# honglianghe/CDNet

Measured on AMD Instinct MI355X. Metric: tiles/sec (train fwd+bwd+Adam), 256x256, higher is better.
Workload: dtype fp32

## Files before the change

cdnet_amd/csrc/conv32.hip:

```cpp
#include <type_traits>
#include "common.h"
#include "conv_args.h"
#include "launch.h"
#include <stdlib.h>

using namespace cdnet;

typedef __attribute__((ext_vector_type(8))) __bf16 bf16x8;
typedef __attribute__((ext_vector_type(2))) __bf16 bf16x2;
typedef __attribute__((ext_vector_type(16))) float f32x16;
typedef __attribute__((ext_vector_type(2))) float f32x2;
typedef unsigned u32x4 __attribute__((ext_vector_type(4)));
typedef float f32x4 __attribute__((ext_vector_type(4)));

namespace {

__device__ __forceinline__ void split8(const float *v, u32x4 &hi, u32x4 &lo) {
#pragma unroll
    for (int k = 0; k < 4; ++k) {
        const f32x2 x = {v[2 * k], v[2 * k + 1]};
        const bf16x2 h = __builtin_convertvector(x, bf16x2);
        const unsigned hb = __builtin_bit_cast(unsigned, h);
        const f32x2 hf = {__builtin_bit_cast(float, hb << 16), __builtin_bit_cast(float, hb & 0xffff0000u)};
        const bf16x2 l = __builtin_convertvector(x - hf, bf16x2);
// ... 328 lines not shown
                        const float v = acc[mi][ni][r];
                        ssum[ni] += v;
                        ssq[ni] = fmaf(v, v, ssq[ni]);
                    }
            } else {
#pragma unroll
            for (int mi = 0; mi < MPW; ++mi)
#pragma unroll
                for (int r = 0; r < 16; ++r) {
                    const int m = (wm * MPW + mi) * 32 + (r & 3) + 8 * (r >> 2) + 4 * half;
                    const float v = ((y0 + m / TW) < A.H && (x0 + m % TW) < A.W) ? acc[mi][ni][r] : 0.f;
                    ssum[ni] += v;
                    ssq[ni] = fmaf(v, v, ssq[ni]);
                }
            }
            ssum[ni] += __shfl_xor(ssum[ni], 32);
            ssq[ni] += __shfl_xor(ssq[ni], 32);
            if (half == 0) {
                s_stats[wave][0][(wn * NPW + ni) * 32 + l31] = ssum[ni];
                s_stats[wave][1][(wn * NPW + ni) * 32 + l31] = ssq[ni];
            }
        }
        __syncthreads();
        if (tid < 2 * BN) {
            const int which = tid / BN, col = tid % BN;
            const int wn_of = col / (NPW * 32);
            float v = 0.f;
#pragma unroll
            for (int k = 0; k < WM; ++k) v += s_stats[k * WN + wn_of][which][col];
            const int co = cout0 + col;
            if (co < A.Cout) A.stats[((size_t)tile * 2 + which) * A.Cout + co] = v;
        }
    }
    store_tile_f32<MPW, NPW, TW>(A, acc, n, y0, x0, wm * MPW, wn * NPW, half, l31, cout0, par >> 1, par & 1);
}

template <int TH, int TW, int BN, int WM, int WN, int TAPS>
int launch_conv32(const ConvArgs &A, hipStream_t st) {
    using L = Lds32<TH, TW, BN, TAPS>;
    int ctot = 0;
    for (int i = 0; i < A.nsrc; ++i) ctot += A.src[i].C;
    const int smem = L::bytes(ctot);
    dim3 grid(cdiv(A.W, TW) * cdiv(A.H, TH) * A.N * A.npar, cdiv(A.Cout, BN), 1);
    return launch_lds<conv_f32_kernel<TH, TW, BN, WM, WN, TAPS>>(grid, 256, L::bytes(XF_MAX), smem, st, "hipFuncSetAttribute(conv32)", "conv_f32_kernel", A);
}

template <int TAPS>
int dispatch_conv32(const ConvArgs &A, hipStream_t st) {
    if (A.tile == 16 && A.BN == 64) return launch_conv32<16, 16, 64, 4, 1, TAPS>(A, st);
    if (A.tile == 16 && A.BN == 32) return launch_conv32<16, 16, 32, 4, 1, TAPS>(A, st);
    if (A.tile == 8 && A.BN == 64) return launch_conv32<8, 8, 64, 2, 2, TAPS>(A, st);
    set_error("cdnet_conv_forward(f32): unsupported configuration tile=%d CK=%d BN=%d", A.tile, A.CK, A.BN);
    return CDNET_E_ARG;
}

template <int BN, int NCH, bool XF, bool ERES>
__global__ __launch_bounds__(256, 4) void conv1x1_f32_stream_kernel(ConvArgs A) {
    constexpr int NPW = BN / 32;
    constexpr int B_PLANE = CK * BN * 2;
    constexpr int CIN = NCH * CK;
    __shared__ __attribute__((aligned(16))) unsigned char smem[NCH * 2 * B_PLANE + 2 * CIN * 4];
    unsigned char *lds_b = smem;
    float *s_xf = reinterpret_cast<float *>(smem + NCH * 2 * B_PLANE);

    const int tid = threadIdx.x, lane = tid & 63, wave = __builtin_amdgcn_readfirstlane(tid >> 6);
    const int half = lane >> 5, l31 = lane & 31;
    const int cout_tile = blockIdx.y, cout0 = cout_tile * BN;
    const ConvSrc &S = A.src[0];
    {
        const u32x4 *wsrc = reinterpret_cast<const u32x4 *>(A.w + (size_t)cout_tile * NCH * B_PLANE);
        u32x4 *bdst = reinterpret_cast<u32x4 *>(lds_b);
        for (int v = tid; v < NCH * 2 * B_PLANE / 16; v += 256) bdst[v] = wsrc[v];
        for (int c = tid; c < CIN; c += 256) {
            s_xf[c] = S.scale ? S.scale[c] : 1.f;
            s_xf[CIN + c] = S.shift ? S.shift[c] : 0.f;
        }
    }
    __syncthreads();

    const size_t P = (size_t)A.N * A.H * A.W;
    const int nblk = (int)((P + 31) / 32), bstride = (int)gridDim.x * 4;
    int blk = (int)blockIdx.x * 4 + wave;
    if (blk >= nblk) return;
    const bool relu = S.relu != 0, orelu = A.orelu != 0, eres_relu = A.eres_relu != 0;
    const int cout = A.Cout;
    const int bbase = half * BN * 16 + l31 * 16;

    float osc[NPW], osh[NPW], esc[NPW], esh[NPW];
#pragma unroll
    for (int ni = 0; ni < NPW; ++ni) {
        const int co = cout0 + ni * 32 + l31, c = co < A.Cout ? co : 0;
        osc[ni] = A.oscale ? A.oscale[c] : 1.f;
        osh[ni] = fmaf(A.bias ? A.bias[c] : 0.f, osc[ni], A.oshift ? A.oshift[c] : 0.f);
        esc[ni] = (ERES && A.eres_scale) ? A.eres_scale[c] : 1.f;
        esh[ni] = (ERES && A.eres_shift) ? A.eres_shift[c] : 0.f;
    }

    const char *xbase = reinterpret_cast<const char *>(S.x);
    char *obase = reinterpret_cast<char *>(A.out) + (size_t)A.out_coff * 4;
    const char *ebase = ERES ? reinterpret_cast<const char *>(A.eres) : xbase;
    const unsigned cs4 = (unsigned)A.out_cstride * 4, ce4 = (unsigned)cout * 4;
    const unsigned vo_in = l31 * (CIN * 4) + half * 32;
    unsigned vo_out[NPW], vo_eres[NPW];
#pragma unroll
    for (int ni = 0; ni < NPW; ++ni) {
        const unsigned co = cout0 + ni * 32 + l31;
// ... 154 lines not shown
        auto xf = [&](float4 v, const float4 *r) {
            v.x = fmaf(v.x, sc.x, sh.x); v.y = fmaf(v.y, sc.y, sh.y); v.z = fmaf(v.z, sc.z, sh.z); v.w = fmaf(v.w, sc.w, sh.w);
            if (r) { v.x += r->x; v.y += r->y; v.z += r->z; v.w += r->w; }
            if (relu) { v.x = fmaxf(v.x, 0.f); v.y = fmaxf(v.y, 0.f); v.z = fmaxf(v.z, 0.f); v.w = fmaxf(v.w, 0.f); }
            return v;
        };
        if (ys >= 0 && ys < Hl && xs >= 0 && xs < Wl) {
            if (!s.pool) {
                const size_t e = img + (size_t)ys * rs + (size_t)xs * s.C + c;
                const float4 raw = *reinterpret_cast<const float4 *>(sx + e);
                if (sr) { const float4 r = *reinterpret_cast<const float4 *>(sr + e); val = xf(raw, &r); }
                else val = xf(raw, nullptr);
            } else {
                float4 raw[4];
                bool ok[4];
#pragma unroll
                for (int q = 0; q < 4; ++q) {
                    int yy = 2 * ys + (q >> 1), xx = 2 * xs + (q & 1);
                    ok[q] = q == 0 || (yy < s.Hs && xx < s.Ws);
                    yy = yy < s.Hs ? yy : s.Hs - 1;
                    xx = xx < s.Ws ? xx : s.Ws - 1;
                    raw[q] = *reinterpret_cast<const float4 *>(sx + img + (size_t)yy * rs + (size_t)xx * s.C + c);
                }
#pragma unroll
                for (int q = 0; q < 4; ++q) {
                    const float4 t = xf(raw[q], nullptr);
                    if (q == 0) val = t;
                    else if (ok[q]) { val.x = fmaxf(val.x, t.x); val.y = fmaxf(val.y, t.y); val.z = fmaxf(val.z, t.z); val.w = fmaxf(val.w, t.w); }
                }
            }
        }
        *reinterpret_cast<float4 *>(out + pix * s.C + c) = val;
    }
}

}

namespace cdnet {

int conv_forward_f32(const ConvArgs &A, hipStream_t st) {
    CDNET_REQUIRE(A.CK == 16, "cdnet_conv_forward(f32): CK must be 16 (got %d)", A.CK);
    for (int i = 0; i < A.nsrc; ++i)
        CDNET_REQUIRE(!A.src[i].pool, "cdnet_conv_forward(f32): pooled sources must be materialised (cdnet_src_materialize)");
    CDNET_REQUIRE(!A.out_f16, "cdnet_conv_forward(f32): out_f16 must be 0");
    {
        const int rc = conv_forward_f32_ws(A, st);
        if (rc >= 0) return rc;
    }
    CDNET_REQUIRE(A.ws != 2, "cdnet_conv_forward(f32): the BatchNorm-backward statistics epilogue (ws = 2) needs the producer / consumer kernel "
                             "(ask cdnet_conv_ws_eligible first)");
    CDNET_REQUIRE(A.taps1 == 0 || A.taps1 == A.taps, "cdnet_conv_forward(f32): a one-tap second source runs on conv_ws32_kernel only (ask cdnet_conv_ws_eligible)");
    CDNET_REQUIRE(!A.pool_out, "cdnet_conv_forward(f32): the fused max-pool output rides in conv_ws32_kernel's epilogue only (ask cdnet_conv_ws_eligible)");
    if (A.taps == 9) return dispatch_conv32<9>(A, st);
    if (A.taps == 4) return dispatch_conv32<4>(A, st);
    {
        const int rc = try_conv1x1_stream(A, st);
        if (rc >= 0) return rc;
    }
    return dispatch_conv32<1>(A, st);
}

int materialize_f32(const ConvSrc &s, int N, int H, int W, void *out, hipStream_t st) {
    const size_t total = (size_t)N * H * W * (s.C / 4);
    size_t g = (total + 255) / 256;
    g = g > 8192 ? 8192 : g;
    materialize_f32_kernel<<<(int)g, 256, 0, st>>>(s, N, H, W, reinterpret_cast<float *>(out));
    return check_launch("cdnet_src_materialize(f32)");
}

}
```

cdnet_amd/csrc/conv_args.h:

```cpp
#pragma once
#include "../../include/cdnet_hip.h"

struct ConvSrc {
    const unsigned short *x;
    const unsigned short *res;
    const float *scale;
    const float *shift;
    int C, Hs, Ws, pool, relu, off_y, off_x;
    int f16, row_stride;
};

struct ConvArgs {
    ConvSrc src[2];
    int nsrc;
    const unsigned short *w;
    const float *bias;
    const float *oscale;
    const float *oshift;
    int orelu;
    unsigned short *out;
    int Cout, out_cstride, out_coff;
    float *stats;
    int N, H, W;
    int taps, npar, ostride, nchunk;
    int tile, CK, BN;
    int out_f16;
    int debug;
    int ws;
    int f32;
    const unsigned short *eres;
    const float *eres_scale, *eres_shift;
    int eres_f16, eres_relu;
    int taps1, pad_;
    unsigned short *pool_out;
    const float *dot_w, *dot_b;
    float *dot_out;
};

enum : int {
    CONV_DBG_WS16_QUAD = 16,
    CONV_DBG_ONE_TILE = 32,
    CONV_DBG_PERSIST_SMALL = 64,
    CONV_DBG_OLD_WS16 = 128,
    CONV_DBG_NO_STREAM_1X1 = 256,
    CONV_DBG_GRID_SHIFT = 8,
};
enum : int {
    WGRAD_DBG_NO_WS = 8,
    WGRAD_DBG_ALL_QUADS = 16,
};

static_assert(sizeof(ConvSrc) == sizeof(cdnet_conv_src), "ConvSrc layout");
static_assert(sizeof(ConvArgs) == sizeof(cdnet_conv_args), "ConvArgs layout");

namespace cdnet {
int conv_forward_f32(const ConvArgs &A, hipStream_t st);
int conv_forward_f32_ws(const ConvArgs &A, hipStream_t st, bool dry_run = false);
int conv_forward_ws16(const ConvArgs &A, hipStream_t st, bool dry_run = false);
int materialize_f32(const ConvSrc &s, int N, int H, int W, void *out, hipStream_t st);
}
```

cdnet_amd/csrc/conv.hip:

```cpp
#include <type_traits>
#include <vector>
#include "common.h"
#include "conv_args.h"
#include "launch.h"
#include "xform.h"
#include "stage16.h"
#include <stdlib.h>

using namespace cdnet;

typedef __attribute__((ext_vector_type(16))) float f32x16;
typedef __attribute__((ext_vector_type(4))) float f32x4;

namespace {

__device__ int g_dbg_dummy;

struct PackDesc {
    const float *w;
    unsigned short *out;
    int Cout, Cin, KH, KW, CK, BN, nchunk, ntile, TAPS, mode, parity;
    unsigned block0, nblocks;
    int split;
    const float *scale;
};

__device__ __forceinline__ void pack_range(const PackDesc &d, size_t first, size_t stride) {
    const float *__restrict__ w = d.w;
    unsigned short *__restrict__ out = d.out;
    const int Cout = d.Cout, Cin = d.Cin, KH = d.KH, KW = d.KW, CK = d.CK, BN = d.BN, nchunk = d.nchunk, TAPS = d.TAPS, mode = d.mode,
              parity = d.parity;
    const size_t total = (size_t)d.ntile * nchunk * TAPS * (CK / 16) * 2 * BN * (d.split ? 2 : 1);
    for (size_t i = first; i < total; i += stride) {
        size_t r = i;
        int tap = r % TAPS; r /= TAPS;
        int col = r % BN; r /= BN;
        int half = r % 2; r /= 2;
        int kc = r % (CK / 16); r /= (CK / 16);
        int hl = 0;
        if (d.split) { hl = r % 2; r /= 2; }
        int chunk = r % nchunk; r /= nchunk;
        int tile = (int)r;
        int co = tile * BN + col;
        const size_t ovec = ((((((size_t)tile * nchunk + chunk) * (d.split ? 2 : 1) + hl) * TAPS + tap) * (CK / 16) + kc) * 2 + half) * BN + col;
        unsigned short o8[8];
#pragma unroll
        for (int j = 0; j < 8; ++j) {
        int ci = chunk * CK + kc * 16 + half * 8 + j;
        float v = 0.f;
        if (co < Cout && ci < Cin) {
            if (mode == 0) {
                v = w[(((size_t)co * Cin + ci) * KH + tap / KW) * KW + tap % KW];
            } else if (mode == 1) {
                int kh = KH - 1 - tap / KW, kw = KW - 1 - tap % KW;
                v = w[(((size_t)ci * Cout + co) * KH + kh) * KW + kw];
            } else if (mode == 2) {
                int a = parity >> 1, b = parity & 1, ty = tap >> 1, tx = tap & 1;
                int kh = a == 0 ? (ty == 0 ? 1 : 3) : (ty == 0 ? 0 : 2);
                int kw = b == 0 ? (tx == 0 ? 1 : 3) : (tx == 0 ? 0 : 2);
                v = w[(((size_t)ci * Cout + co) * 4 + kh) * 4 + kw];
            } else if (mode == 3) {
                int a = parity >> 1, b = parity & 1;
                v = w[(((size_t)ci * Cout + co) * 2 + a) * 2 + b];
            } else if (mode == 7) {
                const int Ct = Cout / 4;
                const int a = co / (2 * Ct), b = (co / Ct) & 1, c = co % Ct;
                const int tf = 8 - tap;
                const int kh = 2 * (tf / 3 - 1) + a + 1, kw = 2 * (tf % 3 - 1) + b + 1;
                if (kh >= 0 && kh < 3 && kw >= 0 && kw < 3) v = w[(((size_t)ci * Ct + c) * 3 + kh) * 3 + kw];
            } else {
                const int Ct = Cin / 4;
                const int a = ci / (2 * Ct), b = (ci / Ct) & 1, c = ci % Ct;
                if (mode == 4) {
                    const int kh = 2 * (tap / 3) + a - 1, kw = 2 * (tap % 3) + b - 1;
                    if (kh >= 0 && kh < 4 && kw >= 0 && kw < 4) v = w[(((size_t)co * Ct + c) * 4 + kh) * 4 + kw];
                } else if (mode == 5) {
                    v = w[(((size_t)co * Ct + c) * 2 + a) * 2 + b];
                } else {
                    const int kh = 2 * (tap / 3 - 1) + a + 1, kw = 2 * (tap % 3 - 1) + b + 1;
                    if (kh >= 0 && kh < 3 && kw >= 0 && kw < 3) v = w[(((size_t)co * Ct + c) * 3 + kh) * 3 + kw];
                }
            }
        }
        if (d.scale && co < Cout) v *= d.scale[co];
        const unsigned short hi = f2bf(v);
        o8[j] = hl ? f2bf(v - bf2f(hi)) : hi;
        }
        uint4 ov;
        ov.x = o8[0] | ((unsigned)o8[1] << 16); ov.y = o8[2] | ((unsigned)o8[3] << 16);
        ov.z = o8[4] | ((unsigned)o8[5] << 16); ov.w = o8[6] | ((unsigned)o8[7] << 16);
        reinterpret_cast<uint4 *>(out)[ovec] = ov;
    }
}

__global__ void pack_weights_kernel(PackDesc d) {
    pack_range(d, (size_t)blockIdx.x * blockDim.x + threadIdx.x, (size_t)gridDim.x * blockDim.x);
}

__global__ void pack_weights_batch_kernel(const PackDesc *__restrict__ table, int n) {
    int lo = 0, hi = n - 1;
    while (lo < hi) {
        const int mid = (lo + hi + 1) >> 1;
        if (table[mid].block0 <= blockIdx.x) lo = mid; else hi = mid - 1;
    }
    const PackDesc d = table[lo];
    pack_range(d, (size_t)(blockIdx.x - d.block0) * blockDim.x + threadIdx.x, (size_t)d.nblocks * blockDim.x);
}

__device__ __forceinline__ V16 max8(V16 a, V16 b, bool nonneg) {
    V16 o;
    if (nonneg) {
        o.u = __builtin_bit_cast(uint4, xf_max_nonneg_bf8(__builtin_bit_cast(xf_u32x4, a.u), __builtin_bit_cast(xf_u32x4, b.u)));
        return o;
    }
#pragma unroll
    for (int j = 0; j < 8; ++j) o.h[j] = bf2f(a.h[j]) >= bf2f(b.h[j]) ? a.h[j] : b.h[j];
    return o;
}

constexpr int XF_MAX = 2048;

__device__ __forceinline__ void load_chan_xf(ChanXf &t, const ConvSrc &s, const float *xf, int xfs, int c) {
    t.on = s.scale != nullptr;
    if (!t.on) return;
    const float4 *ps = reinterpret_cast<const float4 *>(xf ? xf + c : s.scale + c);
    const float4 *ph = reinterpret_cast<const float4 *>(xf ? xf + xfs + c : s.shift + c);
    float4 a = ps[0], b = ps[1], cc = ph[0], d = ph[1];
    t.sc[0] = a.x; t.sc[1] = a.y; t.sc[2] = a.z; t.sc[3] = a.w; t.sc[4] = b.x; t.sc[5] = b.y; t.sc[6] = b.z; t.sc[7] = b.w;
    t.sh[0] = cc.x; t.sh[1] = cc.y; t.sh[2] = cc.z; t.sh[3] = cc.w; t.sh[4] = d.x; t.sh[5] = d.y; t.sh[6] = d.z; t.sh[7] = d.w;
}

template <int TH, int CK>
struct HaloImg {
    static constexpr bool SWZ = (TH == 16 && CK == 16);
    static constexpr int PSTR = SWZ ? CK * 2 : CK * 2 + 16;
    __device__ __forceinline__ static int off(int pix, int hy, int slot) { return pix * PSTR + (SWZ ? ((slot ^ (hy & 1)) * 16) : slot * 16); }
};

template <int TH, int TW, int CK>
__device__ __forceinline__ void stage_input(const ConvSrc &s, int cc0, int n, int y0, int x0, int H, int W,
                                            unsigned char *lds_a, int tid, const float *xf = nullptr, int xfs = 0) {
    constexpr int VPP = CK / 8;
    constexpr int HW_ = TW + 2, NPIX = (TH + 2) * (TW + 2);
    const int slot = tid % VPP;
    ChanXf t;
    load_chan_xf(t, s, xf, xfs, cc0 + slot * 8);
    const bool relu = s.relu != 0;
    const bool f16 = s.f16 != 0;
    const bool plain = !t.on && !relu && s.res == nullptr && !f16;
    const int Hl = s.pool ? (s.Hs + (s.pool == 2)) / 2 : s.Hs, Wl = s.pool ? (s.Ws + (s.pool == 2)) / 2 : s.Ws;
    const size_t rs = s.row_stride ? (size_t)s.row_stride : (size_t)s.Ws * s.C;
    const size_t img = (size_t)n * s.Hs * rs;
    for (int v = tid; v < NPIX * VPP; v += 256) {
        const int pix = v / VPP;
        const int hy = pix / HW_, hx = pix - hy * HW_;
        const int y = y0 - 1 + hy, x = x0 - 1 + hx;
        V16 val;
        val.u = make_uint4(0, 0, 0, 0);
        const int ys = y - s.off_y, xs = x - s.off_x;
// ... 1056 lines not shown
__global__ __launch_bounds__(256) void materialize_kernel(const ConvSrc s, int N, int H, int W, unsigned short *__restrict__ out) {
    const int VPP = s.C / 8;
    const size_t total = (size_t)N * H * W * VPP;
    const bool relu = s.relu != 0, f16 = s.f16 != 0;
    const int Hl = s.pool ? (s.Hs + (s.pool == 2)) / 2 : s.Hs, Wl = s.pool ? (s.Ws + (s.pool == 2)) / 2 : s.Ws;
    const size_t rs = s.row_stride ? (size_t)s.row_stride : (size_t)s.Ws * s.C;
    for (size_t i = (size_t)blockIdx.x * 256 + threadIdx.x; i < total; i += (size_t)gridDim.x * 256) {
        const int slot = (int)(i % VPP);
        const size_t pix = i / VPP;
        const int x = (int)(pix % W), y = (int)((pix / W) % H), n = (int)(pix / ((size_t)W * H));
        ChanXf t;
        load_chan_xf(t, s, nullptr, 0, slot * 8);
        const bool plain = !t.on && !relu && s.res == nullptr && !f16;
        const size_t img = (size_t)n * s.Hs * rs;
        V16 val;
        val.u = make_uint4(0, 0, 0, 0);
        const int ys = y - s.off_y, xs = x - s.off_x;
        if (ys >= 0 && ys < Hl && xs >= 0 && xs < Wl) {
            if (!s.pool) {
                const size_t e = img + (size_t)ys * rs + (size_t)xs * s.C + slot * 8;
                V16 raw;
                raw.u = *reinterpret_cast<const uint4 *>(s.x + e);
                if (plain) val = raw;
                else if (s.res) { V16 r; r.u = *reinterpret_cast<const uint4 *>(s.res + e); val = xform8(raw, &r, t, relu, f16); }
                else val = xform8(raw, nullptr, t, relu, f16);
            } else {
                V16 raw[4];
                bool ok[4];
#pragma unroll
                for (int q = 0; q < 4; ++q) {
                    int yy = 2 * ys + (q >> 1), xx = 2 * xs + (q & 1);
                    ok[q] = q == 0 || (yy < s.Hs && xx < s.Ws);
                    yy = yy < s.Hs ? yy : s.Hs - 1;
                    xx = xx < s.Ws ? xx : s.Ws - 1;
                    raw[q].u = *reinterpret_cast<const uint4 *>(s.x + img + (size_t)yy * rs + (size_t)xx * s.C + slot * 8);
                }
#pragma unroll
                for (int q = 0; q < 4; ++q) {
                    const V16 tv = plain ? raw[q] : xform8(raw[q], nullptr, t, relu, f16);
                    val = q == 0 ? tv : (ok[q] ? max8(val, tv, relu) : val);
                }
            }
        }
        *reinterpret_cast<uint4 *>(out + pix * s.C + slot * 8) = val.u;
    }
}

}

extern "C" size_t cdnet_conv_packed_weight_elems(int Cout, int Cin_padded_chunks, int taps, int CK, int BN, int npar) {
    return (size_t)npar * cdiv(Cout, BN) * Cin_padded_chunks * taps * CK * BN;
}

static int fill_pack_desc(PackDesc &d, const float *w, void *packed, int Cout, int Cin, int KH, int KW, int CK, int BN, int mode, int p,
                          const char *who) {
    const int split = (mode & 16) ? 1 : 0;
    mode &= 15;
    CDNET_REQUIRE(w && packed, "%s: null pointer", who);
    CDNET_REQUIRE(CK % 16 == 0 && BN % 32 == 0 && Cin % CK == 0 && mode >= 0 && mode <= 7, "%s: Cin=%d CK=%d BN=%d mode=%d", who, Cin, CK, BN, mode);
    const int taps = mode == 2 ? 4 : (mode == 3 ? 1 : ((mode == 4 || mode == 6 || mode == 7) ? 9 : (mode == 5 ? 1 : KH * KW)));
    const int nchunk = Cin / CK, ntile = cdiv(Cout, BN);
    const size_t per = (size_t)ntile * nchunk * taps * CK * BN * (split ? 2 : 1);
    d.split = split;
    d.scale = nullptr;
    d.w = w; d.out = (unsigned short *)packed + (size_t)p * per;
    d.Cout = Cout; d.Cin = Cin; d.KH = KH; d.KW = KW; d.CK = CK; d.BN = BN; d.nchunk = nchunk; d.ntile = ntile; d.TAPS = taps; d.mode = mode;
    d.parity = p;
    d.block0 = 0;
    d.nblocks = (unsigned)((per + 2047) / 2048);
    if (d.nblocks > 4096) d.nblocks = 4096;
    return CDNET_OK;
}

extern "C" int cdnet_pack_conv_weights(const float *w, void *packed, int Cout, int Cin, int KH, int KW, int CK, int BN,
                                       int mode, void *stream) {
    const int npar = ((mode & 15) == 2 || (mode & 15) == 3) ? 4 : 1;
    for (int p = 0; p < npar; ++p) {
        PackDesc d;
        int rc = fill_pack_desc(d, w, packed, Cout, Cin, KH, KW, CK, BN, mode, p, "cdnet_pack_conv_weights");
        if (rc) return rc;
        pack_weights_kernel<<<d.nblocks, 256, 0, (hipStream_t)stream>>>(d);
    }
    return check_launch("cdnet_pack_conv_weights");
}

extern "C" int cdnet_pack_conv_weights_scaled(const float *w, const float *cout_scale, void *packed, int Cout, int Cin, int KH, int KW, int CK,
                                              int BN, int mode, void *stream) {
    CDNET_REQUIRE(cout_scale && (mode & 15) == 0, "cdnet_pack_conv_weights_scaled: forward Conv2d packs (mode 0) with a scale vector");
    PackDesc d;
    int rc = fill_pack_desc(d, w, packed, Cout, Cin, KH, KW, CK, BN, mode, 0, "cdnet_pack_conv_weights_scaled");
    if (rc) return rc;
    d.scale = cout_scale;
    pack_weights_kernel<<<d.nblocks, 256, 0, (hipStream_t)stream>>>(d);
    return check_launch("cdnet_pack_conv_weights_scaled");
}

extern "C" size_t cdnet_pack_batch_table_bytes(int n_jobs) { return (size_t)n_jobs * 4 * sizeof(PackDesc); }

extern "C" int cdnet_pack_conv_weights_batch(const cdnet_pack_job *jobs, int n_jobs, void *table, size_t table_bytes, int upload,
                                             void *stream) {
    CDNET_REQUIRE(jobs && n_jobs > 0 && table, "cdnet_pack_conv_weights_batch: null pointer / no jobs");
    CDNET_REQUIRE(table_bytes >= cdnet_pack_batch_table_bytes(n_jobs), "cdnet_pack_conv_weights_batch: table too small");
    static thread_local std::vector<PackDesc> host;
    host.clear();
    unsigned blocks = 0;
    for (int j = 0; j < n_jobs; ++j) {
        const cdnet_pack_job &J = jobs[j];
        const int npar = ((J.mode & 15) == 2 || (J.mode & 15) == 3) ? 4 : 1;
        for (int p = 0; p < npar; ++p) {
            PackDesc d;
            int rc = fill_pack_desc(d, J.w, J.packed, J.Cout, J.Cin, J.KH, J.KW, J.CK, J.BN, J.mode, p, "cdnet_pack_conv_weights_batch");
            if (rc) return rc;
            d.block0 = blocks;
            blocks += d.nblocks;
            host.push_back(d);
        }
    }
    hipStream_t st = (hipStream_t)stream;
    if (upload) {
        if (hipMemcpyAsync(table, host.data(), host.size() * sizeof(PackDesc), hipMemcpyHostToDevice, st) != hipSuccess ||
            hipStreamSynchronize(st) != hipSuccess)
            return check_launch("cdnet_pack_conv_weights_batch(upload)");
    }
    pack_weights_batch_kernel<<<blocks, 256, 0, st>>>((const PackDesc *)table, (int)host.size());
    return check_launch("cdnet_pack_conv_weights_batch");
}

extern "C" int cdnet_conv_forward(const cdnet_conv_args *args, void *stream) {
    CDNET_REQUIRE(args, "cdnet_conv_forward: null args");
    const ConvArgs &A = *reinterpret_cast<const ConvArgs *>(args);
    CDNET_REQUIRE(A.nsrc >= 1 && A.nsrc <= 2 && A.w && (A.out || A.dot_out), "cdnet_conv_forward: bad pointers / nsrc=%d", A.nsrc);
    CDNET_REQUIRE(!A.dot_out || (A.dot_w && !A.f32 && !A.pool_out), "cdnet_conv_forward: dot_out needs dot_w, the 16-bit path and no pool_out");
    CDNET_REQUIRE(A.N > 0 && A.H > 0 && A.W > 0 && A.Cout > 0 && A.Cout % 8 == 0, "cdnet_conv_forward: bad size (Cout must be a multiple of 8)");
    {
        int ctot_xf = 0;
        for (int i = 0; i < A.nsrc; ++i) ctot_xf += A.src[i].C;
        CDNET_REQUIRE(ctot_xf <= XF_MAX, "cdnet_conv_forward: %d source channels exceed the %d-entry scale/shift table", ctot_xf, XF_MAX);
    }
    CDNET_REQUIRE(A.ws == 0 || A.ws == 2, "cdnet_conv_forward: ws must be 0 or 2 (BatchNorm-backward statistics epilogue)");
    if (A.f32) {
        CDNET_REQUIRE(A.f32 == 1, "cdnet_conv_forward: f32 must be 0 or 1");
        for (int i = 0; i < A.nsrc; ++i)
            CDNET_REQUIRE(A.src[i].f16 == 2, "cdnet_conv_forward(f32): every source must be fp32 (f16 = 2)");
    } else {
        for (int i = 0; i < A.nsrc; ++i)
            CDNET_REQUIRE(A.src[i].f16 == 0 || A.src[i].f16 == 1, "cdnet_conv_forward: fp32 sources need args.f32 = 1");
    }
    if (A.eres && A.ws != 2) {
        CDNET_REQUIRE(A.ostride == 1 && A.npar == 1 && A.out_coff == 0 && A.out_cstride == A.Cout && !A.stats && !A.orelu &&
                      !A.out_f16 && ((A.eres_scale == nullptr) == (A.eres_shift == nullptr)),
                      "cdnet_conv_forward: fused residual epilogue needs a dense bf16 output, no statistics and no ReLU before the add");
    }
    int nchunk = 0;
    for (int i = 0; i < A.nsrc; ++i) {
        CDNET_REQUIRE(A.src[i].x && A.src[i].C % A.CK == 0, "cdnet_conv_forward: source %d channels %d not a multiple of CK=%d",
                      i, A.src[i].C, A.CK);
        CDNET_REQUIRE(!(A.src[i].pool && A.src[i].res), "cdnet_conv_forward: pool+residual source unsupported");
        nchunk += A.src[i].C / A.CK;
    }
    const bool padded = A.nchunk == nchunk + 1 && A.taps == 9 && A.nsrc == 2 && !A.f32;
    CDNET_REQUIRE(nchunk == A.nchunk || padded, "cdnet_conv_forward: nchunk %d != %d", A.nchunk, nchunk);
    CDNET_REQUIRE((A.taps == 9 && A.npar == 1 && A.ostride == 1) || (A.taps == 1 && A.npar == 1 && A.ostride == 1) ||
                  (A.taps == 4 && A.npar == 4 && A.ostride == 2) || (A.taps == 1 && A.npar == 4 && A.ostride == 2),
                  "cdnet_conv_forward: taps=%d npar=%d ostride=%d", A.taps, A.npar, A.ostride);
// ... 54 lines not shown
```

include/cdnet_hip.h:

```cpp
#ifndef CDNET_HIP_H
#define CDNET_HIP_H

#include <stddef.h>
#include <stdint.h>

#ifdef __cplusplus
extern "C" {
#endif

#define CDNET_OK            0
#define CDNET_E_ARG         1
#define CDNET_E_WORKSPACE   2
#define CDNET_E_LAUNCH      3

#define CDNET_ABI_VERSION   5

int         cdnet_abi_version(void);
size_t      cdnet_abi_sizeof(const char *struct_name);
const char *cdnet_last_error(void);
const char *cdnet_build_info(void);
int         cdnet_spin(int microseconds, void *stream);
int         cdnet_box_copy(const void *src, void *dst, size_t bytes, void *stream);
int         cdnet_box_mfma(const uint32_t *seed, float *sink, unsigned long long *stamps, int workgroups, int waves_per_wg, int iters, void *stream);

// ... 35 lines not shown
                             float *prob, uint8_t *pred, uint8_t *fill, uint8_t *small, int32_t *label, int32_t *final_, int32_t *counts,
                             void *stream);
int cdnet_dilate_labels(const int32_t *label, int N, int H, int W, int radius, int32_t *out, void *stream);


typedef struct cdnet_conv_src {
    const uint16_t *x;
    const uint16_t *res;
    const float *scale;
    const float *shift;
    int C;
    int Hs, Ws;
    int pool;
    int relu;
    int off_y, off_x;
    int f16;
    int row_stride;
} cdnet_conv_src;

typedef struct cdnet_conv_args {
    cdnet_conv_src src[2];
    int nsrc;
    const uint16_t *w;
    const float *bias;
    const float *oscale;
    const float *oshift;
    int orelu;
    uint16_t *out;
    int Cout, out_cstride, out_coff;
    float *stats;
    int N, H, W;
    int taps;
    int npar;
    int ostride;
    int nchunk;
    int tile, CK, BN;
    int out_f16;
    int debug;
    int ws;
    int f32;
    const uint16_t *eres;
    const float *eres_scale, *eres_shift;
    int eres_f16, eres_relu;
    int taps1;
    int pad_;
    uint16_t *pool_out;
    const float *dot_w;
    const float *dot_b;
    float *dot_out;
} cdnet_conv_args;

size_t cdnet_conv_packed_weight_elems(int Cout, int nchunk, int taps, int CK, int BN, int npar);
#define CDNET_PACK_SPLIT 16
int cdnet_pack_conv_weights(const float *w, void *packed, int Cout, int Cin, int KH, int KW, int CK, int BN, int mode,
                            void *stream);
int cdnet_pack_conv_weights_scaled(const float *w, const float *cout_scale, void *packed, int Cout, int Cin, int KH, int KW, int CK,
                                   int BN, int mode, void *stream);
typedef struct cdnet_pack_job {
    const float *w;
    void *packed;
    int Cout, Cin, KH, KW, CK, BN, mode, pad_;
} cdnet_pack_job;
size_t cdnet_pack_batch_table_bytes(int n_jobs);
int cdnet_pack_conv_weights_batch(const cdnet_pack_job *jobs, int n_jobs, void *table, size_t table_bytes, int upload,
                                  void *stream);
int cdnet_conv_forward(const cdnet_conv_args *args, void *stream);

int cdnet_input_pack(const float *x, int N, int C, int H, int W, void *out_bf16_nhwc16, void *stream);
int cdnet_input_pack_f32(const float *x, int N, int C, int H, int W, float *out_f32_nhwc16, void *stream);
int cdnet_bn_fold_eval(const float *gamma, const float *beta, const float *running_mean, const float *running_var,
                       const float *conv_bias, float eps, int C, float *scale, float *shift, void *stream);
int cdnet_bn_finalize_train(const float *stats, int T, int C, float count, const float *gamma, const float *beta,
                            const float *conv_bias, float eps, float momentum, float *running_mean,
                            float *running_var, float *scale, float *shift, float *save_mean, float *save_invstd,
                            void *stream);

typedef struct cdnet_head_feat {
    const uint16_t *raw;
    const uint16_t *res;
    const float *scale;
    const float *shift;
    int relu;
    int f16;
} cdnet_head_feat;

#define CDNET_HEAD_WEIGHT_FLOATS 855
int cdnet_dam_head_forward(const cdnet_head_feat *f1, const cdnet_head_feat *f2, const cdnet_head_feat *f3,
                           const float *head_weights, int N, int H, int W, float *mask, float *point,
                           float *direction, void *stream);
int cdnet_final_conv1x1(const cdnet_head_feat *f, const float *w, const float *b, int K, int N, int H, int W,
                        float *out, void *stream);
size_t cdnet_bias_grad_workspace_floats(int C);
int cdnet_bias_grad(const uint16_t *grad_out, size_t npix, int C, float *workspace, size_t workspace_floats, float *db, void *stream);
int cdnet_bias_grad_f32(const float *grad_out, size_t npix, int C, float *workspace, size_t workspace_floats, float *db, void *stream);
size_t cdnet_final_conv1x1_backward_workspace_floats(void);
int cdnet_final_conv1x1_backward(const cdnet_head_feat *f, const float *w, const float *dlogits, int K, int N, int H, int W,
                                 uint16_t *df, float *workspace, size_t workspace_floats, float *dw, float *db, void *stream);

int cdnet_conv_ws_eligible(const cdnet_conv_args *args);

int cdnet_src_materialize(const cdnet_conv_src *src, int N, int H, int W, uint16_t *out, void *stream);

size_t cdnet_conv_wgrad_slab_floats(int C_src, int Cout, int taps, int npar, int ci_tiles, int ksplit);
int cdnet_conv_backward_weight(const cdnet_conv_src *src, int src_coff, int Csrc_real, int Cin_real,
                               const uint16_t *grad_out, int Cout, int N, int H, int W, int taps, int npar,
                               int ostride, int ci_tiles, int ksplit, float *slab, float *dw, int mode, void *stream);
// ... 158 lines not shown
```

Baseline: 1108.

## Add fused persistent kernel computing all four transposed-conv parities per tile

Adds a persistent 1024-thread kernel for the stride-2 transposed convolution (4 taps, 4 parities). Each input tile is staged once in LDS and shared by all four output parities, instead of being reloaded once per parity. The next item's global loads are prefetched into registers while the current chunk computes, and BatchNorm statistics and the interleaved stride-2 output store are done in the epilogue. The cost is a large LDS footprint and a single block per CU, which limits occupancy and latency hiding.

```diff
diff --git a/cdnet_amd/csrc/conv32.hip b/cdnet_amd/csrc/conv32.hip
--- a/cdnet_amd/csrc/conv32.hip
+++ b/cdnet_amd/csrc/conv32.hip
@@ -404,6 +404,262 @@
     if (A.tile == 8 && A.BN == 64) return launch_conv32<8, 8, 64, 2, 2, TAPS>(A, st);
     set_error("cdnet_conv_forward(f32): unsupported configuration tile=%d CK=%d BN=%d", A.tile, A.CK, A.BN);
     return CDNET_E_ARG;
+}
+
+template <int BN>
+struct LdsT4 {
+    static constexpr int NPIX = 18 * 18;
+    static constexpr int A_PLANE = NPIX * PSTR;
+    static constexpr int B_PLANE = 4 * CK * BN * 2;
+    static constexpr int STAGE = 2 * A_PLANE + 4 * 2 * B_PLANE;
+    static constexpr int STATS_BYTES = 4 * 4 * 2 * BN * 4 + 4 * 4 * 2 * (BN / 32) * 64 * 4;
+    static constexpr int MAIN = ((STAGE > STATS_BYTES ? STAGE : STATS_BYTES) + 15) / 16 * 16;
+    static int bytes(int ctot) { return MAIN + 2 * ((ctot + 7) / 8 * 8) * 4; }
+};
+
+template <int BN>
+__global__ __launch_bounds__(1024) void convt4_f32_fused_kernel(ConvArgs A) {
+    using L = LdsT4<BN>;
+    constexpr int TW = 16, HW_ = 18, NPIX = L::NPIX;
+    constexpr int NT = 1024, NPW = BN / 32;
+    constexpr int VPP = CK / 8;
+    constexpr int NBP = 2 * L::B_PLANE / 16;
+    constexpr int NB = 4 * NBP / NT;
+    static_assert(NPIX * VPP <= NT && NBP * 2 % NT == 0 && NT % NBP == 0, "staging");
+
+    extern __shared__ __attribute__((aligned(16))) unsigned char smem[];
+    unsigned char *lds_a = smem;
+    unsigned char *lds_b = smem + 2 * L::A_PLANE;
+    float (*s_stats)[4][2][BN] = reinterpret_cast<float (*)[4][2][BN]>(smem);
+    float (*s_part)[4][2][NPW][64] = reinterpret_cast<float (*)[4][2][NPW][64]>(smem + 4 * 4 * 2 * BN * 4);
+    float *s_xf = reinterpret_cast<float *>(smem + L::MAIN);
+
+    const int tid = threadIdx.x, lane = tid & 63, wave = __builtin_amdgcn_readfirstlane(tid >> 6);
+    const int blk = wave & 7, ra = wave >> 3;
+    const int half = lane >> 5, l31 = lane & 31;
+    const ConvSrc &S = A.src[0];
+    const int ctot = S.C, xfs = (ctot + 7) / 8 * 8;
+    for (int c = tid; c < ctot; c += NT) {
+        s_xf[c] = S.scale ? S.scale[c] : 1.f;
+        s_xf[xfs + c] = S.shift ? S.shift[c] : 0.f;
+    }
+
+    const int tiles_x = (A.W + 15) / 16, tiles_y = (A.H + 15) / 16;
+    const int tiles_img = tiles_x * tiles_y;
+    const int NC = (A.Cout + BN - 1) / BN, T = tiles_img * A.N * NC;
+    struct Item { int n, rt, y0, x0, cout_tile, eoff; };
+    const int slot = tid % VPP, hy = (tid / VPP) / HW_, hx = (tid / VPP) - hy * HW_;
+    const size_t rs = S.row_stride ? (size_t)S.row_stride : (size_t)S.Ws * S.C;
+    auto item = [&](int lin) {
+        const int q = T >> 3, rem = T & 7;
+        const int xcd = lin & 7, idx = lin >> 3;
+        const int seq = xcd < rem ? xcd * (q + 1) + idx : rem * (q + 1) + (xcd - rem) * q + idx;
+        Item it;
+        const int tile = seq / NC;
+        it.cout_tile = seq - tile * NC;
+        it.n = tile / tiles_img;
+        it.rt = tile - it.n * tiles_img;
+        const int ty_ = it.rt / tiles_x;
+        it.y0 = ty_ * 16;
+        it.x0 = (it.rt - ty_ * tiles_x) * 16;
+        const int y = it.y0 - 1 + hy, x = it.x0 - 1 + hx;
+        const bool ok = tid < NPIX * VPP && (unsigned)y < (unsigned)A.H && (unsigned)x < (unsigned)A.W;
+        it.eoff = ok ? y * (int)rs + x * S.C + slot * 8 : -1;
+        return it;
+    };
+
+    f32x4 pa[2];
+    u32x4 pb[NB];
+    auto issue = [&](const Item &it, int chunk) {
+        const float *base = reinterpret_cast<const float *>(S.x) + (size_t)it.n * S.Hs * rs + chunk * CK;
+        const f32x4 *p = reinterpret_cast<const f32x4 *>(base + (it.eoff >= 0 ? it.eoff : 0));
+        pa[0] = p[0];
+        pa[1] = p[1];
+#pragma unroll
+        for (int i = 0; i < NB; ++i) {
+            const int v = tid + i * NT;
+            const u32x4 *wsrc = reinterpret_cast<const u32x4 *>(A.w + ((size_t)((v / NBP) * NC + it.cout_tile) * A.nchunk + chunk) * L::B_PLANE);
+            pb[i] = wsrc[v % NBP];
+        }
+    };
+    auto commit = [&](const Item &it, int chunk) {
+        u32x4 *bdst = reinterpret_cast<u32x4 *>(lds_b);
+#pragma unroll
+        for (int i = 0; i < NB; ++i) bdst[tid + i * NT] = pb[i];
+        if (tid >= NPIX * VPP) return;
+        const bool on = S.scale != nullptr, relu = S.relu != 0;
+        const float *xf = s_xf + chunk * CK + slot * 8;
+        u32x4 hi = {0u, 0u, 0u, 0u}, lo = {0u, 0u, 0u, 0u};
+        if (it.eoff >= 0) {
+            float v[8] = {pa[0][0], pa[0][1], pa[0][2], pa[0][3], pa[1][0], pa[1][1], pa[1][2], pa[1][3]};
+            if (on) {
+#pragma unroll
+                for (int j = 0; j < 8; ++j) v[j] = fmaf(v[j], xf[j], xf[xfs + j]);
+            }
+            if (relu) {
+#pragma unroll
+                for (int j = 0; j < 8; ++j) v[j] = fmaxf(v[j], 0.f);
+            }
+            split8(v, hi, lo);
+        }
+        unsigned char *d = lds_a + (tid / VPP) * PSTR + slot * 16;
+        *reinterpret_cast<u32x4 *>(d) = hi;
+        *reinterpret_cast<u32x4 *>(d + L::A_PLANE) = lo;
+    };
+
+    const int abase = ((blk * 2 + ra + l31 / TW) * HW_ + l31 % TW) * PSTR + half * 16;
+    const int bbase = ra * 4 * L::B_PLANE + half * BN * 16 + l31 * 16;
+    const int G = (int)gridDim.x;
+
+    int lin = (int)blockIdx.x;
+    Item cur = item(lin), nxt = cur;
+    issue(cur, 0);
+    for (;;) {
+        f32x16 acc[2][NPW];
+#pragma unroll
+        for (int b = 0; b < 2; ++b)
+#pragma unroll
+            for (int ni = 0; ni < NPW; ++ni)
+#pragma unroll
+                for (int r = 0; r < 16; ++r) acc[b][ni][r] = 0.f;
+        const bool more = lin + G < T;
+        for (int chunk = 0; chunk < A.nchunk; ++chunk) {
+            __syncthreads();
+            commit(cur, chunk);
+            __syncthreads();
+            if (chunk + 1 < A.nchunk) issue(cur, chunk + 1);
+            else if (more) {
+                nxt = item(lin + G);
+                issue(nxt, 0);
+            }
+#pragma unroll
+            for (int pos = 0; pos < 6; ++pos) {
+                const int dy = 1 - pos / 3, c = 2 - pos % 3;
+                const bf16x8 ah = *reinterpret_cast<const bf16x8 *>(lds_a + abase + (dy * HW_ + c) * PSTR);
+                const bf16x8 al = *reinterpret_cast<const bf16x8 *>(lds_a + L::A_PLANE + abase + (dy * HW_ + c) * PSTR);
+#pragma unroll
+                for (int b = 0; b < 2; ++b) {
+                    const int dx = c - b;
+                    if (dx < 0 || dx > 1) continue;
+                    const int t = (1 - dy) * 2 + (1 - dx);
+#pragma unroll
+                    for (int ni = 0; ni < NPW; ++ni) {
+                        const bf16x8 bh = *reinterpret_cast<const bf16x8 *>(lds_b + b * 2 * L::B_PLANE + bbase + t * 2 * BN * 16 + ni * 512);
+                        const bf16x8 bl = *reinterpret_cast<const bf16x8 *>(lds_b + b * 2 * L::B_PLANE + L::B_PLANE + bbase + t * 2 * BN * 16 + ni * 512);
+                        acc[b][ni] = __builtin_amdgcn_mfma_f32_32x32x16_bf16(al, bh, acc[b][ni], 0, 0, 0);
+                        acc[b][ni] = __builtin_amdgcn_mfma_f32_32x32x16_bf16(ah, bl, acc[b][ni], 0, 0, 0);
+                        acc[b][ni] = __builtin_amdgcn_mfma_f32_32x32x16_bf16(ah, bh, acc[b][ni], 0, 0, 0);
+                    }
+                }
+            }
+        }
+
+        const int n = cur.n, y0 = cur.y0, x0 = cur.x0;
+        const int cout0 = cur.cout_tile * BN;
+        const bool full_tile = y0 + 16 <= A.H && x0 + 16 <= A.W;
+        if (A.stats) {
+            __syncthreads();
+            const int pair = blk >> 1;
+#pragma unroll
+            for (int step = 0; step < 2; ++step) {
+                if ((blk & 1) == step) {
+#pragma unroll
+                    for (int b = 0; b < 2; ++b)
+#pragma unroll
+                        for (int ni = 0; ni < NPW; ++ni) {
+                            const int p = 2 * ra + b;
+                            float ssum = step ? s_part[p][pair][0][ni][lane] : 0.f, ssq = step ? s_part[p][pair][1][ni][lane] : 0.f;
+#pragma unroll
+                            for (int r = 0; r < 16; ++r) {
+                                const int m = blk * 32 + (r & 3) + 8 * (r >> 2) + 4 * half;
+                                const float v = (full_tile || ((y0 + m / TW) < A.H && (x0 + m % TW) < A.W)) ? acc[b][ni][r] : 0.f;
+                                ssum += v;
+                                ssq = fmaf(v, v, ssq);
+                            }
+                            if (step == 0) {
+                                s_part[p][pair][0][ni][lane] = ssum;
+                                s_part[p][pair][1][ni][lane] = ssq;
+                            } else {
+                                ssum += __shfl_xor(ssum, 32);
+                                ssq += __shfl_xor(ssq, 32);
+                                if (half == 0) {
+                                    s_stats[p][pair][0][ni * 32 + l31] = ssum;
+                                    s_stats[p][pair][1][ni * 32 + l31] = ssq;
+                                }
+                            }
+                        }
+                }
+                __syncthreads();
+            }
+            if (tid < 4 * 2 * BN) {
+                const int p = tid / (2 * BN), which = (tid / BN) & 1, col = tid % BN;
+                float v = 0.f;
+#pragma unroll
+                for (int k = 0; k < 4; ++k) v += s_stats[p][k][which][col];
+                const int co = cout0 + col;
+                const int row = (n * 4 + p) * tiles_img + cur.rt;
+                if (co < A.Cout) A.stats[((size_t)row * 2 + which) * A.Cout + co] = v;
+            }
+        }
+        const int Wo = A.W * 2, cs = A.out_cstride;
+        const bool pack16 = A.Cout <= 16;
+        float *tb = reinterpret_cast<float *>(A.out) + (((size_t)n * A.H * 2 + 2 * y0 + 4 * blk + ra) * Wo + 2 * x0) * cs + A.out_coff +
+                    (pack16 ? (8 * half + (l31 >> 4)) * cs + (l31 & 15) : half * cs);
+#pragma unroll
+        for (int ni = 0; ni < NPW; ++ni) {
+            const int co = cout0 + ni * 32 + l31;
+            const bool cok = co < A.Cout;
+            const float osc = (A.oscale && cok) ? A.oscale[co] : 1.f;
+            const float osh = fmaf((A.bias && cok) ? A.bias[co] : 0.f, osc, (A.oshift && cok) ? A.oshift[co] : 0.f);
+            auto epi = [&](float x) {
+                float v = fmaf(x, osc, osh);
+                if (A.orelu) v = fmaxf(v, 0.f);
+                return v;
+            };
+#pragma unroll
+            for (int r = 0; r < 16; ++r) {
+                const int ml = (r & 3) + 8 * (r >> 2);
+                const int yl = blk * 2 + ml / TW;
+                const float v0 = epi(acc[0][ni][r]), v1 = epi(acc[1][ni][r]);
+                const int roff = (2 * (ml / TW) * Wo + 2 * (ml % TW)) * cs;
+                if (pack16) {
+                    const int xl = ml % TW + 4 * half;
+                    const float t = __shfl_xor(v1, 16);
+                    const bool ok = (l31 & 15) < A.Cout && (full_tile || (y0 + yl < A.H && x0 + xl < A.W));
+                    if (ok) tb[roff] = (l31 & 16) ? t : v0;
+                } else {
+                    const float got = __shfl_xor(half ? v0 : v1, 32);
+#pragma unroll
+                    for (int h = 0; h < 2; ++h) {
+                        const int xl = ml % TW + 4 * h;
+                        const float v = h == 0 ? (half ? got : v0) : (half ? v1 : got);
+                        const bool ok = cok && (full_tile || (y0 + yl < A.H && x0 + xl < A.W));
+                        if (ok) tb[roff + 8 * h * cs + co] = v;
+                    }
+                }
+            }
+        }
+        if (!more) break;
+        lin += G;
+        cur = nxt;
+    }
+}
+
+int try_convt4_fused(const ConvArgs &A, hipStream_t st) {
+    if (A.debug & CONV_DBG_NO_FUSED_CONVT) return -1;
+    if (A.taps != 4 || A.taps1 != 0 || A.npar != 4 || A.ostride != 2 || A.ws || A.pool_out || A.eres || A.nsrc != 1) return -1;
+    if (A.tile != 16 || A.BN != 32) return -1;
+    const ConvSrc &s = A.src[0];
+    const long long rs = s.row_stride ? s.row_stride : (long long)s.Ws * s.C;
+    if (s.off_y || s.off_x || s.Hs != A.H || s.Ws != A.W || s.pool || s.res || s.C != A.nchunk * CK || s.C > XF_MAX) return -1;
+    if (rs * s.Hs >= (1LL << 31) || 34LL * A.W * 2 * A.out_cstride >= (1LL << 31)) return -1;
+    int n_cu = 0;
+    if (const int rc = cu_count(&n_cu)) return rc;
+    using L = LdsT4<32>;
+    const long long T = (long long)cdiv(A.W, 16) * cdiv(A.H, 16) * A.N * cdiv(A.Cout, 32);
+    if (T >= (1LL << 31)) return -1;
+    dim3 grid((unsigned)(T < n_cu ? T : n_cu), 1, 1);
+    return launch_lds<convt4_f32_fused_kernel<32>>(grid, 1024, L::bytes(XF_MAX), L::bytes(s.C), st, "hipFuncSetAttribute(convt4 fused)", "convt4_f32_fused_kernel", A);
 }
 
 template <int BN, int NCH, bool XF, bool ERES>
@@ -664,7 +920,11 @@
     CDNET_REQUIRE(A.taps1 == 0 || A.taps1 == A.taps, "cdnet_conv_forward(f32): a one-tap second source runs on conv_ws32_kernel only (ask cdnet_conv_ws_eligible)");
     CDNET_REQUIRE(!A.pool_out, "cdnet_conv_forward(f32): the fused max-pool output rides in conv_ws32_kernel's epilogue only (ask cdnet_conv_ws_eligible)");
     if (A.taps == 9) return dispatch_conv32<9>(A, st);
-    if (A.taps == 4) return dispatch_conv32<4>(A, st);
+    if (A.taps == 4) {
+        const int rc = try_convt4_fused(A, st);
+        if (rc >= 0) return rc;
+        return dispatch_conv32<4>(A, st);
+    }
     {
         const int rc = try_conv1x1_stream(A, st);
         if (rc >= 0) return rc;
diff --git a/cdnet_amd/csrc/conv_args.h b/cdnet_amd/csrc/conv_args.h
--- a/cdnet_amd/csrc/conv_args.h
+++ b/cdnet_amd/csrc/conv_args.h
@@ -43,6 +43,7 @@
     CONV_DBG_PERSIST_SMALL = 64,
     CONV_DBG_OLD_WS16 = 128,
     CONV_DBG_NO_STREAM_1X1 = 256,
+    CONV_DBG_NO_FUSED_CONVT = 512,
     CONV_DBG_GRID_SHIFT = 8,
 };
 enum : int {
```

Measured after the change: 1112, median of 6. Within noise of the previous version (+0.4%).

## Stage weight bricks through LDS for coalesced fp32-to-bf16 weight packing

Applied to the files above, without the earlier changes.

Adds a tiled weight-pack path for modes 0 and 1 without a scale vector. Each block loads a contiguous brick of fp32 weights into shared memory with vectorized float4 reads, then emits packed bf16 output vectors from LDS. In split mode it writes the hi and lo halves from the same pass. The aim is to replace the scattered per-element global gathers of the range packer, which runs every step after Adam updates the weights, at the cost of extra LDS use and new index-mapping code.

```diff
diff --git a/cdnet_amd/csrc/conv.hip b/cdnet_amd/csrc/conv.hip
--- a/cdnet_amd/csrc/conv.hip
+++ b/cdnet_amd/csrc/conv.hip
@@ -5,6 +5,7 @@
 #include "launch.h"
 #include "xform.h"
 #include "stage16.h"
+#include "tile_maps.h"
 #include <stdlib.h>
 
 using namespace cdnet;
@@ -22,6 +23,7 @@
     int Cout, Cin, KH, KW, CK, BN, nchunk, ntile, TAPS, mode, parity;
     unsigned block0, nblocks;
     int split;
+    int tiled;
     const float *scale;
 };
 
@@ -93,18 +95,86 @@
     }
 }
 
-__global__ void pack_weights_kernel(PackDesc d) {
+__device__ __forceinline__ void pack_brick_tiled(const PackDesc &d, unsigned b, float *__restrict__ s_w) {
+    const tmap::PackGeom g = tmap::pack_geom(d.Cout, d.Cin, d.CK, d.BN, d.TAPS, d.mode, d.split);
+    const tmap::PackBrick k = tmap::pack_brick(g, b);
+    const float *__restrict__ w = d.w;
+    const bool wvec = (reinterpret_cast<size_t>(w) & 15) == 0;
+    const int runv = g.run / 4, nv = g.rows * runv;
+    constexpr int NLD = 4;
+    for (int v0 = threadIdx.x; v0 < nv; v0 += NLD * 256) {
+        f32x4 x[NLD];
+#pragma unroll
+        for (int u = 0; u < NLD; ++u) {
+            const int v = v0 + u * 256;
+            x[u] = f32x4{0.f, 0.f, 0.f, 0.f};
+            if (v < nv) {
+                const int row = v / runv, q = (v % runv) * 4;
+                size_t off;
+                int len;
+                tmap::pack_src_run(g, k, row, &off, &len);
+                if (wvec && (off & 3) == 0 && q + 4 <= len) {
+                    x[u] = *reinterpret_cast<const f32x4 *>(w + off + q);
+                } else {
+#pragma unroll
+                    for (int i = 0; i < 4; ++i)
+                        if (q + i < len) x[u][i] = w[off + q + i];
+                }
+            }
+        }
+#pragma unroll
+        for (int u = 0; u < NLD; ++u) {
+            const int v = v0 + u * 256;
+            if (v < nv) {
+                float *o = s_w + (v / runv) * g.pitch + (v % runv) * 4;
+                o[0] = x[u][0]; o[1] = x[u][1]; o[2] = x[u][2]; o[3] = x[u][3];
+            }
+        }
+    }
+    __syncthreads();
+    uint4 *__restrict__ out = reinterpret_cast<uint4 *>(d.out);
+    const size_t img = (size_t)g.TAPS * (g.CK / 8) * g.BN;
+    for (int u = threadIdx.x; u < g.nvec; u += 256) {
+        int col_l, ci_l0, tap;
+        const size_t ovec = tmap::pack_out_vec(g, k, 0, u, &col_l, &ci_l0, &tap);
+        unsigned short h8[8], l8[8];
+#pragma unroll
+        for (int j = 0; j < 8; ++j) {
+            const float v = s_w[tmap::pack_lds_index(g, col_l, ci_l0 + j, tap)];
+            h8[j] = f2bf(v);
+            l8[j] = f2bf(v - bf2f(h8[j]));
+        }
+        uint4 ov;
+        ov.x = h8[0] | ((unsigned)h8[1] << 16); ov.y = h8[2] | ((unsigned)h8[3] << 16);
+        ov.z = h8[4] | ((unsigned)h8[5] << 16); ov.w = h8[6] | ((unsigned)h8[7] << 16);
+        out[ovec] = ov;
+        if (d.split) {
+            ov.x = l8[0] | ((unsigned)l8[1] << 16); ov.y = l8[2] | ((unsigned)l8[3] << 16);
+            ov.z = l8[4] | ((unsigned)l8[5] << 16); ov.w = l8[6] | ((unsigned)l8[7] << 16);
+            out[ovec + img] = ov;
+        }
+    }
+}
+
+__global__ __launch_bounds__(256) void pack_weights_kernel(PackDesc d) {
     pack_range(d, (size_t)blockIdx.x * blockDim.x + threadIdx.x, (size_t)gridDim.x * blockDim.x);
 }
 
-__global__ void pack_weights_batch_kernel(const PackDesc *__restrict__ table, int n) {
+__global__ __launch_bounds__(256) void pack_weights_tiled_kernel(PackDesc d) {
+    __shared__ float s_w[tmap::PACK_LDS_FLOATS];
+    pack_brick_tiled(d, blockIdx.x, s_w);
+}
+
+__global__ __launch_bounds__(256) void pack_weights_batch_kernel(const PackDesc *__restrict__ table, int n) {
+    __shared__ float s_w[tmap::PACK_LDS_FLOATS];
     int lo = 0, hi = n - 1;
     while (lo < hi) {
         const int mid = (lo + hi + 1) >> 1;
         if (table[mid].block0 <= blockIdx.x) lo = mid; else hi = mid - 1;
     }
     const PackDesc d = table[lo];
-    pack_range(d, (size_t)(blockIdx.x - d.block0) * blockDim.x + threadIdx.x, (size_t)d.nblocks * blockDim.x);
+    if (d.tiled) pack_brick_tiled(d, blockIdx.x - d.block0, s_w);
+    else pack_range(d, (size_t)(blockIdx.x - d.block0) * blockDim.x + threadIdx.x, (size_t)d.nblocks * blockDim.x);
 }
 
 __device__ __forceinline__ V16 max8(V16 a, V16 b, bool nonneg) {
@@ -1267,9 +1337,10 @@
     return (size_t)npar * cdiv(Cout, BN) * Cin_padded_chunks * taps * CK * BN;
 }
 
-static int fill_pack_desc(PackDesc &d, const float *w, void *packed, int Cout, int Cin, int KH, int KW, int CK, int BN, int mode, int p,
-                          const char *who) {
-    const int split = (mode & 16) ? 1 : 0;
+static int fill_pack_desc(PackDesc &d, const float *w, const float *scale, void *packed, int Cout, int Cin, int KH, int KW, int CK, int BN,
+                          int mode, int p, const char *who) {
+    const int split = (mode & CDNET_PACK_SPLIT) ? 1 : 0;
+    const bool force_range = (mode & CDNET_PACK_RANGE) != 0;
     mode &= 15;
     CDNET_REQUIRE(w && packed, "%s: null pointer", who);
     CDNET_REQUIRE(CK % 16 == 0 && BN % 32 == 0 && Cin % CK == 0 && mode >= 0 && mode <= 7, "%s: Cin=%d CK=%d BN=%d mode=%d", who, Cin, CK, BN, mode);
@@ -1277,13 +1348,18 @@
     const int nchunk = Cin / CK, ntile = cdiv(Cout, BN);
     const size_t per = (size_t)ntile * nchunk * taps * CK * BN * (split ? 2 : 1);
     d.split = split;
-    d.scale = nullptr;
+    d.scale = scale;
     d.w = w; d.out = (unsigned short *)packed + (size_t)p * per;
     d.Cout = Cout; d.Cin = Cin; d.KH = KH; d.KW = KW; d.CK = CK; d.BN = BN; d.nchunk = nchunk; d.ntile = ntile; d.TAPS = taps; d.mode = mode;
     d.parity = p;
     d.block0 = 0;
     d.nblocks = (unsigned)((per + 2047) / 2048);
     if (d.nblocks > 4096) d.nblocks = 4096;
+    d.tiled = 0;
+    if ((mode == 0 || mode == 1) && !scale && !force_range) {
+        const tmap::PackGeom g = tmap::pack_geom(Cout, Cin, CK, BN, taps, mode, split);
+        if (g.nblocks) { d.tiled = 1; d.nblocks = g.nblocks; }
+    }
     return CDNET_OK;
 }
 
@@ -1292,9 +1368,10 @@
     const int npar = ((mode & 15) == 2 || (mode & 15) == 3) ? 4 : 1;
     for (int p = 0; p < npar; ++p) {
         PackDesc d;
-        int rc = fill_pack_desc(d, w, packed, Cout, Cin, KH, KW, CK, BN, mode, p, "cdnet_pack_conv_weights");
+        int rc = fill_pack_desc(d, w, nullptr, packed, Cout, Cin, KH, KW, CK, BN, mode, p, "cdnet_pack_conv_weights");
         if (rc) return rc;
-        pack_weights_kernel<<<d.nblocks, 256, 0, (hipStream_t)stream>>>(d);
+        if (d.tiled) pack_weights_tiled_kernel<<<d.nblocks, 256, 0, (hipStream_t)stream>>>(d);
+        else pack_weights_kernel<<<d.nblocks, 256, 0, (hipStream_t)stream>>>(d);
     }
     return check_launch("cdnet_pack_conv_weights");
 }
@@ -1303,9 +1380,8 @@
                                               int BN, int mode, void *stream) {
     CDNET_REQUIRE(cout_scale && (mode & 15) == 0, "cdnet_pack_conv_weights_scaled: forward Conv2d packs (mode 0) with a scale vector");
     PackDesc d;
-    int rc = fill_pack_desc(d, w, packed, Cout, Cin, KH, KW, CK, BN, mode, 0, "cdnet_pack_conv_weights_scaled");
+    int rc = fill_pack_desc(d, w, cout_scale, packed, Cout, Cin, KH, KW, CK, BN, mode, 0, "cdnet_pack_conv_weights_scaled");
     if (rc) return rc;
-    d.scale = cout_scale;
     pack_weights_kernel<<<d.nblocks, 256, 0, (hipStream_t)stream>>>(d);
     return check_launch("cdnet_pack_conv_weights_scaled");
 }
@@ -1324,7 +1400,7 @@
         const int npar = ((J.mode & 15) == 2 || (J.mode & 15) == 3) ? 4 : 1;
         for (int p = 0; p < npar; ++p) {
             PackDesc d;
-            int rc = fill_pack_desc(d, J.w, J.packed, J.Cout, J.Cin, J.KH, J.KW, J.CK, J.BN, J.mode, p, "cdnet_pack_conv_weights_batch");
+            int rc = fill_pack_desc(d, J.w, nullptr, J.packed, J.Cout, J.Cin, J.KH, J.KW, J.CK, J.BN, J.mode, p, "cdnet_pack_conv_weights_batch");
             if (rc) return rc;
             d.block0 = blocks;
             blocks += d.nblocks;
diff --git a/cdnet_amd/csrc/tile_maps.h b/cdnet_amd/csrc/tile_maps.h
--- /dev/null
+++ b/cdnet_amd/csrc/tile_maps.h
@@ -0,0 +1,79 @@
+#pragma once
+#include <stddef.h>
+
+#if defined(__HIPCC__)
+#define CDNET_TM_HD __host__ __device__ inline
+#else
+#define CDNET_TM_HD inline
+#endif
+
+namespace cdnet {
+namespace tmap {
+
+enum : int { PACK_BRICK_FLOATS = 9216, PACK_LDS_FLOATS = PACK_BRICK_FLOATS + 128 };
+
+struct PackGeom {
+    int Cout, Cin, CK, BN, nchunk, ntile, TAPS, mode, nimg;
+    int BNs, ncg;
+    int rows, run, pitch;
+    int nvec;
+    unsigned nblocks;
+};
+
+CDNET_TM_HD PackGeom pack_geom(int Cout, int Cin, int CK, int BN, int TAPS, int mode, int split) {
+    PackGeom g;
+    g.Cout = Cout; g.Cin = Cin; g.CK = CK; g.BN = BN; g.TAPS = TAPS; g.mode = mode; g.nimg = split ? 2 : 1;
+    g.nchunk = Cin / CK; g.ntile = (Cout + BN - 1) / BN;
+    int bns = BN;
+    while (bns % 16 == 0 && (long long)bns * CK * TAPS > PACK_BRICK_FLOATS) bns /= 2;
+    g.BNs = bns; g.ncg = BN / bns;
+    g.rows = mode == 0 ? bns : CK;
+    g.run = (mode == 0 ? CK : bns) * TAPS;
+    g.pitch = g.run | 1;
+    g.nvec = TAPS * (CK / 16) * 2 * bns;
+    const bool ok = (mode == 0 || mode == 1) && (long long)g.rows * g.pitch <= PACK_LDS_FLOATS && CK % 16 == 0 && Cin % CK == 0;
+    g.nblocks = ok ? (unsigned)(g.ntile * g.nchunk * g.ncg) : 0u;
+    return g;
+}
+
+struct PackBrick { int tile, chunk, cg; };
+
+CDNET_TM_HD PackBrick pack_brick(const PackGeom &g, unsigned b) {
+    PackBrick k;
+    k.cg = (int)(b % (unsigned)g.ncg); b /= (unsigned)g.ncg;
+    k.chunk = (int)(b % (unsigned)g.nchunk);
+    k.tile = (int)(b / (unsigned)g.nchunk);
+    return k;
+}
+
+CDNET_TM_HD void pack_src_run(const PackGeom &g, const PackBrick &k, int row, size_t *off, int *len) {
+    const int col0 = k.tile * g.BN + k.cg * g.BNs;
+    if (g.mode == 0) {
+        const int co = col0 + row;
+        *off = ((size_t)co * g.Cin + (size_t)k.chunk * g.CK) * g.TAPS;
+        *len = co < g.Cout ? g.run : 0;
+    } else {
+        const int ci = k.chunk * g.CK + row;
+        int n = g.Cout - col0;
+        n = n < 0 ? 0 : (n > g.BNs ? g.BNs : n);
+        *off = ((size_t)ci * g.Cout + col0) * g.TAPS;
+        *len = n * g.TAPS;
+    }
+}
+
+CDNET_TM_HD int pack_lds_index(const PackGeom &g, int col_l, int ci_l, int tap) {
+    return g.mode == 0 ? col_l * g.pitch + ci_l * g.TAPS + tap : ci_l * g.pitch + col_l * g.TAPS + (g.TAPS - 1 - tap);
+}
+
+CDNET_TM_HD size_t pack_out_vec(const PackGeom &g, const PackBrick &k, int img, int u, int *col_l, int *ci_l0, int *tap) {
+    const int c = u % g.BNs, rowo = u / g.BNs;
+    const int kc2 = g.CK / 8;
+    *col_l = c; *ci_l0 = (rowo % kc2) * 8; *tap = rowo / kc2;
+    const size_t block = ((size_t)k.tile * g.nchunk + k.chunk) * g.nimg + img;
+    return (block * g.TAPS * kc2 + rowo) * g.BN + (size_t)k.cg * g.BNs + c;
+}
+
+CDNET_TM_HD size_t pack_total_vecs(const PackGeom &g) { return (size_t)g.ntile * g.nchunk * g.nimg * g.TAPS * (g.CK / 8) * g.BN; }
+
+}
+}
diff --git a/include/cdnet_hip.h b/include/cdnet_hip.h
--- a/include/cdnet_hip.h
+++ b/include/cdnet_hip.h
@@ -111,6 +111,7 @@
 
 size_t cdnet_conv_packed_weight_elems(int Cout, int nchunk, int taps, int CK, int BN, int npar);
 #define CDNET_PACK_SPLIT 16
+#define CDNET_PACK_RANGE 32
 int cdnet_pack_conv_weights(const float *w, void *packed, int Cout, int Cin, int KH, int KW, int CK, int BN, int mode,
                             void *stream);
 int cdnet_pack_conv_weights_scaled(const float *w, const float *cout_scale, void *packed, int Cout, int Cin, int KH, int KW, int CK,
```

Result: no change. 1108 before, 1113 after (median of 6 runs) (+0.5%).
